# techshoww/RoMa

Measured on AMD Instinct MI355X. Metric: image-pairs/sec at 560->864, higher is better.
Workload: dtype fp16; 1 GPU; roma_outdoor 560->864 full coarse-to-fine symmetric match (BASELINE configs[1]; configs[2] = --pairs 8 --gpus 8); launch=eager launches, coarse_res=560, upsample_res=864, parallelism=single GPU

## Files before the change

include/roma_hip.h:

```cpp
#ifndef ROMA_HIP_H
#define ROMA_HIP_H

#include <stdint.h>

#ifdef __cplusplus
extern "C" {
#endif

#define ROMA_ABI_VERSION 5

enum { ROMA_F32 = 0, ROMA_F16 = 1, ROMA_BF16 = 2 };
enum { ROMA_NCHW = 0, ROMA_NHWC = 1 };
enum { ROMA_LC_AUTO = 0, ROMA_LC_TILE8X4 = 1, ROMA_LC_TILE8X8 = 2, ROMA_LC_ROWS8 = 3 };
enum { ROMA_E_ARG = -1, ROMA_E_DTYPE = -2, ROMA_E_SHAPE = -3, ROMA_E_ALIGN = -4, ROMA_E_UNSUPPORTED = -5 };

int roma_abi_version(void);
const char* roma_last_error(void);

int roma_local_corr(const void* f0, const void* f1, const float* flow, void* out,
                    int B, int C, int H, int W, int r, int dtype,
                    int layout, int f0_pitch, int f1_pitch, int out_layout, int out_pitch, int f1_batch_shift, int variant,
                    void* stream);

int roma_warp_bilinear(const void* src, const float* flow, void* dst,
                       int B, int C, int Hs, int Ws, int H, int W, int dtype,
                       int layout, int src_pitch, int dst_layout, int dst_pitch, int src_batch_shift, void* stream);

int roma_disp_emb(const float* flow, const float* weight, const float* bias, void* dst,
                  int B, int E, int H, int W, float gain, int dtype, int dst_layout, int dst_pitch, void* stream);

int roma_interp_bilinear(const float* x, float* y, int N, int Hi, int Wi, int Ho, int Wo, void* stream);

int roma_interp_bilinear_pair(const float* x0, float* y0, int N0, const float* x1, float* y1, int N1, int Hi, int Wi, int Ho, int Wo,
                              void* stream);

int roma_refiner_assemble(const void* src, const float* flow, const float* weight, const float* bias, void* buf, int B, int C, int E,
                          int D, int pitch, int Hs, int Ws, int H, int W, int src_pitch, int src_batch_shift, float gain, int dtype,
                          void* stream);

int roma_flow_update(float* flow, float* cert, const float* cert_in, const float* delta,
                     int B, int H, int W, float sx, float sy, void* stream);

int roma_cls_to_flow_refine(const void* logits, float* flow_out, float* cert_out,
                            int B, int C, int HW, long stride_b, long stride_c, long stride_p,
                            int dtype, void* stream);

int roma_cos_kernel(const void* x, const void* y, float* K, int B, int N, int M, int D, int dtype, int x_pitch, int y_pitch,
                    int y_batch_shift, float T, float eps, float diag_add, void* stream);

int roma_chol_diag_block(float* A, int lda, long strideA, float* W, int ldw, long strideW, int nb, int B, int* info,
                         int info_base, void* stream);

int roma_chol_step(float* A, int lda, long strideA, int n, int ncols, int j, int nb, const float* W, int ldw, long strideW, float* R,
                   int ldr, long strideR, float* Wn, int ldwn, long strideWn, int* info, int info_base, int B, void* stream);

int roma_chol_subst_step(int dir, const float* W, int ldw, long strideW, const float* R, long strideRb, long strideRs, int ldr, float* T,
                         long strideTb, long strideTs, int ldt, int t_in_panel, float* X, int ldx, long strideX, int n, int m, int nb,
                         int s, int B, void* stream);

int roma_attention_fwd(const void* q, const void* k, const void* v, void* o, int B, int H, int Nq, int Nk, int head_dim, long q_sb,
                       long q_sn, long q_sh, long k_sb, long k_sn, long k_sh, long v_sb, long v_sn, long v_sh, long o_sb, long o_sn,
                       long o_sh, float scale, int dtype, void* stream);

int roma_match_finalize(const float* flow, const float* cert, const float* cert16, float* warp, float* certainty,
                        int P, int H, int W, int H16, int W16, int symmetric, void* stream);

int roma_kde_density(const float* x, float* density, int N, int down, float std, int half_mode, void* stream);

int roma_race_keys(const float* p, const long* counter, float* keys, long N, float thresh, unsigned seed, unsigned stage,
                   void* stream);

int roma_nn_argmin(const float* q, const float* r, int* idx, int NQ, int NR, void* stream);

int roma_resample_u8(const void* in, void* out, int H, int W, int C, int out_size, int axis, const int* bounds,
                     const int* coef, int ksize, void* stream);
int roma_normalize_u8(const void* in, float* out, int H, int W, const float* mean3, const float* std3, void* stream);

int roma_bias_relu_nchw(void* x, const void* bias, int B, int C, int HW, int dtype, void* stream);

int roma_bias_relu_pool2_nchw(void* x, const void* bias, void* pooled, int B, int C, int H, int W, int dtype, void* stream);

int roma_bias_relu_nhwc(void* x, const void* bias, long npix, int C, int dtype, void* stream);
int roma_bias_relu_pool2_nhwc(void* x, const void* bias, void* pooled, int B, int C, int H, int W, int dtype, void* stream);

int roma_dwconv5x5_bn_relu(const void* x, const float* w, const float* scale, const float* shift, void* y,
                           int B, int C, int H, int W, int dtype, int x_pitch, int y_pitch, void* stream);

int roma_refiner_block(const void* x, const void* w25, const float* scale, const float* shift, const void* wt,
                       const float* bias, void* y, int B, int C, int H, int W, int kpad, int dtype, int x_pitch, int y_pitch,
                       void* stream);

int roma_refiner_wide_pack(const void* wt, void* wp, int D);
int roma_refiner_wide_taps(const void* w25, void* w25p, int D);
int roma_refiner_block_wide(const void* x, const void* w25p, const float* scale, const float* shift, const void* wp,
                            const float* bias, void* y, int B, int H, int W, int D, int x_pitch, int y_pitch, int dtype,
                            void* stream);

int roma_pointwise_mfma(const void* x, const void* wt, const float* bias, void* y, long M, int C, int kpad, int dtype,
                        int x_pitch, int y_pitch, void* stream);

int roma_refiner_head(const void* x, const float* wo, const float* bo, float* flow, const float* cert_in, float* cert_out,
// ... 76 lines not shown
```

roma_amd/_lib.py:

```python
from __future__ import annotations

import ctypes
import os
from ctypes import c_char_p, c_float, c_int, c_long, c_void_p

_HERE = os.path.dirname(os.path.abspath(__file__))
LIB_PATH = os.path.join(_HERE, "csrc", "libroma_hip.so")

ROMA_F32, ROMA_F16, ROMA_BF16 = 0, 1, 2
ROMA_NCHW, ROMA_NHWC = 0, 1
LC_VARIANTS = {"auto": 0, "tile8x4": 1, "tile8x8": 2, "rows8": 3}
ABI_VERSION = 5
SCORE_MSAC, SCORE_MAGSAC = 0, 1
ROMA_E_ARG, ROMA_E_DTYPE, ROMA_E_SHAPE, ROMA_E_ALIGN, ROMA_E_UNSUPPORTED = -1, -2, -3, -4, -5

SIGNATURES = {
    "roma_abi_version": [],
    "roma_last_error": [],
    "roma_local_corr": [c_void_p, c_void_p, c_void_p, c_void_p, c_int, c_int, c_int, c_int, c_int, c_int,
                        c_int, c_int, c_int, c_int, c_int, c_int, c_int, c_void_p],
    "roma_warp_bilinear": [c_void_p, c_void_p, c_void_p, c_int, c_int, c_int, c_int, c_int, c_int, c_int,
                           c_int, c_int, c_int, c_int, c_int, c_void_p],
    "roma_disp_emb": [c_void_p, c_void_p, c_void_p, c_void_p, c_int, c_int, c_int, c_int, c_float, c_int, c_int, c_int, c_void_p],
    "roma_interp_bilinear": [c_void_p, c_void_p, c_int, c_int, c_int, c_int, c_int, c_void_p],
    "roma_interp_bilinear_pair": [c_void_p, c_void_p, c_int, c_void_p, c_void_p, c_int, c_int, c_int, c_int, c_int, c_void_p],
    "roma_refiner_assemble": [c_void_p, c_void_p, c_void_p, c_void_p, c_void_p, c_int, c_int, c_int, c_int, c_int, c_int, c_int, c_int,
                              c_int, c_int, c_int, c_float, c_int, c_void_p],
    "roma_project_skinny": [c_void_p, c_void_p, c_void_p, c_void_p, c_long, c_int, c_int, c_int, c_int, c_int, c_void_p],
    "roma_flow_update": [c_void_p, c_void_p, c_void_p, c_void_p, c_int, c_int, c_int, c_float, c_float, c_void_p],
    "roma_cls_to_flow_refine": [c_void_p, c_void_p, c_void_p, c_int, c_int, c_int, c_long, c_long, c_long, c_int, c_void_p],
    "roma_cos_kernel": [c_void_p, c_void_p, c_void_p, c_int, c_int, c_int, c_int, c_int, c_int, c_int, c_int, c_float, c_float,
                        c_float, c_void_p],
    "roma_add_layernorm": [c_void_p, c_int, c_long, c_void_p, c_int, c_long, c_void_p, c_void_p, c_void_p, c_void_p, c_int, c_long,
                           c_long, c_int, c_float, c_void_p],
    "roma_attention_fwd": [c_void_p, c_void_p, c_void_p, c_void_p, c_int, c_int, c_int, c_int, c_int] + [c_long] * 12 + [c_float, c_int, c_void_p],
    "roma_chol_diag_block": [c_void_p, c_int, c_long, c_void_p, c_int, c_long, c_int, c_int, c_void_p, c_int, c_void_p],
    "roma_chol_step": [c_void_p, c_int, c_long, c_int, c_int, c_int, c_int, c_void_p, c_int, c_long, c_void_p, c_int, c_long,
                       c_void_p, c_int, c_long, c_void_p, c_int, c_int, c_void_p],
    "roma_chol_subst_step": [c_int, c_void_p, c_int, c_long, c_void_p, c_long, c_long, c_int, c_void_p, c_long, c_long, c_int, c_int,
                             c_void_p, c_int, c_long, c_int, c_int, c_int, c_int, c_int, c_void_p],
    "roma_match_finalize": [c_void_p, c_void_p, c_void_p, c_void_p, c_void_p, c_int, c_int, c_int, c_int, c_int, c_int, c_void_p],
    "roma_kde_density": [c_void_p, c_void_p, c_int, c_int, c_float, c_int, c_void_p],
    "roma_nn_argmin": [c_void_p, c_void_p, c_void_p, c_int, c_int, c_void_p],
    "roma_race_keys": [c_void_p, c_void_p, c_void_p, c_long, c_float, ctypes.c_uint, ctypes.c_uint, c_void_p],
    "roma_dwconv5x5_bn_relu": [c_void_p, c_void_p, c_void_p, c_void_p, c_void_p, c_int, c_int, c_int, c_int, c_int, c_int, c_int, c_void_p],
    "roma_resample_u8": [c_void_p, c_void_p, c_int, c_int, c_int, c_int, c_int, c_void_p, c_void_p, c_int, c_void_p],
    "roma_normalize_u8": [c_void_p, c_void_p, c_int, c_int, c_void_p, c_void_p, c_void_p],
    "roma_bias_relu_nchw": [c_void_p, c_void_p, c_int, c_int, c_int, c_int, c_void_p],
    "roma_bias_relu_pool2_nchw": [c_void_p, c_void_p, c_void_p, c_int, c_int, c_int, c_int, c_int, c_void_p],
    "roma_bias_relu_nhwc": [c_void_p, c_void_p, c_long, c_int, c_int, c_void_p],
    "roma_bias_relu_pool2_nhwc": [c_void_p, c_void_p, c_void_p, c_int, c_int, c_int, c_int, c_int, c_void_p],
    "roma_pointwise_mfma": [c_void_p, c_void_p, c_void_p, c_void_p, c_long, c_int, c_int, c_int, c_int, c_int, c_void_p],
    "roma_refiner_block": [c_void_p, c_void_p, c_void_p, c_void_p, c_void_p, c_void_p, c_void_p, c_int, c_int, c_int, c_int, c_int, c_int,
                           c_int, c_int, c_void_p],
    "roma_refiner_wide_pack": [c_void_p, c_void_p, c_int],
    "roma_refiner_wide_taps": [c_void_p, c_void_p, c_int],
    "roma_jpeg_info": [c_void_p, c_long, c_void_p],
    "roma_jpeg_entropy_decode": [c_void_p, c_long, c_void_p, c_void_p],
    "roma_jpeg_reconstruct": [c_void_p, c_void_p, c_void_p, c_void_p, c_void_p, c_void_p],
    "roma_refiner_block_wide": [c_void_p, c_void_p, c_void_p, c_void_p, c_void_p, c_void_p, c_void_p, c_int, c_int, c_int, c_int, c_int, c_int,
                                c_int, c_void_p],
    "roma_refiner_head": [c_void_p, c_void_p, c_void_p, c_void_p, c_void_p, c_void_p, c_void_p, c_int, c_int, c_int, c_int, c_int, c_int,
                          c_float, c_float, c_void_p],
    "roma_pointwise_small": [c_void_p, c_void_p, c_void_p, c_void_p, c_long, c_int, c_int, c_int, c_int, c_void_p],
    "roma_tiny_corr_posembed": [c_void_p, c_void_p, c_void_p, c_int, c_int, c_int, c_int, c_int, c_int, c_int, c_void_p],
    "roma_ransac_workspace": [c_int, c_int, c_int, c_int, c_void_p],
    "roma_ransac_hypotheses": [c_int, c_void_p, c_void_p, c_int, c_int, c_int, c_float, ctypes.c_uint, c_int, c_void_p, c_long, c_void_p],
    "roma_ransac_select": [c_int, c_void_p, c_void_p, c_int, c_int, c_int, c_float, c_int, c_void_p, c_long, c_void_p, c_void_p,
                           c_void_p],
    "roma_ransac_hypotheses_ex": [c_int, c_void_p, c_void_p, c_int, c_int, c_int, c_float, c_int, ctypes.c_uint, c_int, c_void_p, c_long,
                                  c_void_p],
    "roma_ransac_select_ex": [c_int, c_void_p, c_void_p, c_int, c_int, c_int, c_float, c_int, c_int, c_void_p, c_long, c_void_p, c_void_p,
                              c_void_p],
    "roma_magsac_table": [c_void_p, c_void_p],
    "roma_essential_workspace": [c_int, c_int, c_int, c_void_p],
    "roma_essential_hypotheses": [c_void_p, c_void_p, c_void_p, c_void_p, c_int, c_int, c_int, c_float, ctypes.c_uint, c_int, c_void_p,
                                  c_long, c_void_p],
    "roma_essential_select": [c_void_p, c_void_p, c_void_p, c_void_p, c_int, c_int, c_int, c_float, c_int, c_void_p, c_long, c_void_p,
                              c_void_p, c_void_p],
    "roma_essential_hypotheses_ex": [c_void_p, c_void_p, c_void_p, c_void_p, c_int, c_int, c_int, c_float, c_int, ctypes.c_uint, c_int,
                                     c_void_p, c_long, c_void_p],
    "roma_essential_select_ex": [c_void_p, c_void_p, c_void_p, c_void_p, c_int, c_int, c_int, c_float, c_int, c_int, c_void_p, c_long,
                                 c_void_p, c_void_p, c_void_p],
    "roma_recover_pose": [c_void_p, c_void_p, c_void_p, c_void_p, c_void_p, c_void_p, c_int, c_int, c_void_p, c_void_p, c_void_p,
                          c_void_p, c_void_p],
# ... 48 lines not shown
```

roma_amd/csrc/cos_kernel.hip:

```cpp
#include "common.h"

namespace roma {
namespace {

typedef float f32x16 __attribute__((ext_vector_type(16)));
constexpr int BT = 64, KT = 16, LD = KT + 1;

template <typename T> __device__ __forceinline__ float4_t ld4(const T* p) {
  if constexpr (sizeof(T) == 4) {
    return *reinterpret_cast<const float4_t*>(p);
  } else {
    typedef T v4 __attribute__((ext_vector_type(4)));
    const v4 h = *reinterpret_cast<const v4*>(p);
    return float4_t{(float)h[0], (float)h[1], (float)h[2], (float)h[3]};
  }
}

template <typename T>
__global__ __launch_bounds__(256) void cos_kernel_mfma(const T* __restrict__ x, const T* __restrict__ y, float* __restrict__ K,
                                                       int N, int M, int D, int x_pitch, int y_pitch, int y_shift, float invT,
                                                       float eps, float diag_add) {
  __shared__ float sA[BT * LD], sB[BT * LD];
  __shared__ double sN[2 * BT];
  const int tid = threadIdx.x, lane = tid & 63, wave = tid >> 6;
  const int wr = wave >> 1, wc = wave & 1;
  const int b = blockIdx.z, n0 = blockIdx.y * BT, m0 = blockIdx.x * BT;
  const T* xb = x + (size_t)b * N * x_pitch;
  const T* yb = y + (size_t)((b + y_shift) % (int)gridDim.z) * M * y_pitch;
  f32x16 acc;
  double accd[16];
#pragma unroll
  for (int i = 0; i < 16; ++i) { acc[i] = 0.f; accd[i] = 0.0; }
  double nrm = 0.0;
  const int lr = tid >> 2, lc = (tid & 3) * 4;
  for (int k0 = 0; k0 < D; k0 += KT) {
    float4_t va{0, 0, 0, 0}, vb{0, 0, 0, 0};
    if (n0 + lr < N) va = ld4<T>(xb + (size_t)(n0 + lr) * x_pitch + k0 + lc);
    if (m0 + lr < M) vb = ld4<T>(yb + (size_t)(m0 + lr) * y_pitch + k0 + lc);
    __syncthreads();
#pragma unroll
    for (int i = 0; i < 4; ++i) {
      sA[lr * LD + lc + i] = va[i];
      sB[lr * LD + lc + i] = vb[i];
    }
    __syncthreads();
    if (tid < 2 * BT) {
      const float* r = (tid < BT ? sA : sB) + (tid & (BT - 1)) * LD;
#pragma unroll
      for (int i = 0; i < KT; ++i) nrm = __builtin_fma((double)r[i], (double)r[i], nrm);
    }
    const float* pa = sA + (wr * 32 + (lane & 31)) * LD + (lane >> 5);
    const float* pb = sB + (wc * 32 + (lane & 31)) * LD + (lane >> 5);
#pragma unroll
    for (int kk = 0; kk < KT; kk += 2) acc = __builtin_amdgcn_mfma_f32_32x32x2f32(pa[kk], pb[kk], acc, 0, 0, 0);
    if (((k0 / KT) & 3) == 3 || k0 + KT >= D) {
#pragma unroll
      for (int i = 0; i < 16; ++i) { accd[i] += (double)acc[i]; acc[i] = 0.f; }
    }
  }
  if (tid < 2 * BT) sN[tid] = sqrt(nrm);
  __syncthreads();
  const int col = lane & 31;
  const int m = m0 + wc * 32 + col;
  const double ny = sN[BT + wc * 32 + col];
#pragma unroll
  for (int r = 0; r < 16; ++r) {
    const int row = (r & 3) + 8 * (r >> 2) + 4 * (lane >> 5);
    const int n = n0 + wr * 32 + row;
    if (n < N && m < M) {
      const double c = accd[r] / (sN[wr * 32 + row] * ny + (double)eps);
      float v = (float)exp((c - 1.0) * (double)invT);
      if (n == m) v += diag_add;
      K[((size_t)b * N + n) * M + m] = v;
    }
  }
}

}
}

using namespace roma;

extern "C" int roma_cos_kernel(const void* x, const void* y, float* K, int B, int N, int M, int D, int dtype, int x_pitch,
                               int y_pitch, int y_batch_shift, float T, float eps, float diag_add, void* stream) {
  ROMA_REQUIRE(x && y && K, ROMA_E_ARG, "roma_cos_kernel: null pointer");
  ROMA_REQUIRE(B > 0 && N > 0 && M > 0 && D > 0, ROMA_E_SHAPE, "roma_cos_kernel: bad shape");
  ROMA_REQUIRE(D % KT == 0, ROMA_E_SHAPE, "roma_cos_kernel: D=%d must be a multiple of %d", D, KT);
  ROMA_REQUIRE(x_pitch >= D && y_pitch >= D, ROMA_E_SHAPE, "roma_cos_kernel: row pitch smaller than D");
  ROMA_REQUIRE(dtype >= ROMA_F32 && dtype <= ROMA_BF16, ROMA_E_DTYPE, "roma_cos_kernel: unknown dtype %d", dtype);
  const int e16 = dtype == ROMA_F32 ? 4 : 8;
  ROMA_REQUIRE(aligned16(x) && aligned16(y) && x_pitch % e16 == 0 && y_pitch % e16 == 0, ROMA_E_ALIGN,
               "roma_cos_kernel: x and y must be 16-byte aligned with row pitches that keep every row 16-byte aligned");
  ROMA_REQUIRE(y_batch_shift >= 0 && y_batch_shift < B, ROMA_E_ARG, "roma_cos_kernel: y_batch_shift %d outside [0, B)", y_batch_shift);
  ROMA_REQUIRE(T > 0.f, ROMA_E_ARG, "roma_cos_kernel: temperature must be positive");
  dim3 grid((M + BT - 1) / BT, (N + BT - 1) / BT, B);
  hipStream_t s = static_cast<hipStream_t>(stream);
#define ROMA_COS(TT)                                                                                                         \
  hipLaunchKernelGGL((cos_kernel_mfma<TT>), grid, dim3(256), 0, s, (const TT*)x, (const TT*)y, K, N, M, D, x_pitch, y_pitch, \
                     y_batch_shift, 1.f / T, eps, diag_add)
  if (dtype == ROMA_F32) ROMA_COS(float); else if (dtype == ROMA_F16) ROMA_COS(half_t); else ROMA_COS(bf16_t);
#undef ROMA_COS
  ROMA_CHECK_LAUNCH();
}
```

roma_amd/matcher.py:

```python
from __future__ import annotations

import math
import os
from collections import namedtuple
from typing import Dict, Optional
from warnings import warn

import numpy as np
import torch
import torch.nn as nn
import torch.nn.functional as F

from . import ops
from .transformer import Block, TransformerDecoder

IMAGENET_MEAN = (0.485, 0.456, 0.406)
IMAGENET_STD = (0.229, 0.224, 0.225)


def pixel_grid(b, h, w, device):
    ys = torch.linspace(-1 + 1 / h, 1 - 1 / h, h, device=device)
    xs = torch.linspace(-1 + 1 / w, 1 - 1 / w, w, device=device)
    return torch.stack((xs[None, :].expand(h, w), ys[:, None].expand(h, w)), dim=0)[None].expand(b, 2, h, w).contiguous()

# ... 160 lines not shown
                cur = cur.view(B, h, w, Dp)
        return cur, P

    @torch.no_grad()
    def forward(self, x, y, flow, scale_factor=1, logits=None, dtype=None):
        flow = flow.float().contiguous()
        cur, P = self._body(x, y, flow, scale_factor, dtype or self.amp_dtype)
        B, h, w, Dp = cur.shape
        out = torch.addmm(P.bo, cur.reshape(B * h * w, Dp).float(), P.wo)
        out = out.view(B, h, w, self.out_dim).permute(0, 3, 1, 2).contiguous()
        return out[:, :-1], out[:, -1:]

    @torch.no_grad()
    def forward_update(self, x, y, flow, certainty, scale_factor, sx, sy, dtype=None, buf=None, batch_shift=0):
        cur, P = self._body(x, y, flow, scale_factor, dtype or self.amp_dtype, buf=buf, batch_shift=batch_shift)
        return ops.refiner_head(cur, P.wo, P.bo, flow, certainty, sx, sy)


class CosKernel(nn.Module):
    def __init__(self, T=0.2, learn_temperature=False):
        super().__init__()
        self.T = T

    def __call__(self, x, y, eps=1e-6):
        return ops.cos_kernel(x, y, T=self.T, eps=eps)


class GP(nn.Module):

    def __init__(self, gp_dim=512, T=0.2, sigma_noise=0.1, kernel=None, **_):
        super().__init__()
        self.K = CosKernel(T=T)
        self.sigma_noise = sigma_noise
        self.pos_conv = nn.Conv2d(2, gp_dim, 1, 1)
        self.dim = gp_dim
        self._basis = {}

    def basis(self, b, h, w, device):
        key = (h, w, device, _params_version(self.pos_conv))
        f = self._basis.get(key)
        if f is None:
            g = pixel_grid(1, h, w, device)
            f = torch.cos(8 * math.pi * F.conv2d(g, self.pos_conv.weight.float(), self.pos_conv.bias.float()))
            f = f.flatten(2).transpose(1, 2).contiguous()
            self._basis = {key: f}
        return f.expand(b, -1, -1)

    @torch.no_grad()
    def forward(self, x, y, **kwargs):
        b, c, h1, w1 = x.shape
        _, _, h2, w2 = y.shape
        xs = x.float().flatten(2).transpose(1, 2).contiguous()
        ys = y.float().flatten(2).transpose(1, 2).contiguous()
        K_yy = ops.cos_kernel(ys, ys, T=self.K.T, diag_add=self.sigma_noise)
        K_xy = ops.cos_kernel(xs, ys, T=self.K.T)
        mu = self.posterior_product(K_xy, ops.spd_solve(K_yy, self.basis(1, h2, w2, x.device)))
        return mu.transpose(1, 2).reshape(b, self.dim, h1, w1)

    def posterior_rows(self, xs, ys, h2, w2, fp64=False, batch_shift=0, out=None, check="now"):
        B, n = xs.shape[0], xs.shape[1]
        s = batch_shift % B
        basis = self.basis(1, h2, w2, xs.device)
        if fp64:
            a = xs.double()
            c = (a.roll(-s, 0) if s else a) if ys is None else ys.double()

            def cosk(u, v):
                g = torch.einsum("bnd,bmd->bnm", u, v) / (u.norm(dim=-1)[..., None] * v.norm(dim=-1)[:, None] + 1e-6)
                return ((g - 1.0) / self.K.T).exp()

            Kyy = cosk(c, c) + self.sigma_noise * torch.eye(c.shape[1], device=c.device, dtype=torch.float64)
            Z = torch.cholesky_solve(basis.double().expand(B, -1, -1), torch.linalg.cholesky(Kyy))
            mu = (cosk(a, c) @ Z).float()
            if out is not None:
                out.copy_(mu)
                return out
            return mu
        if ys is None:
            K_self = ops.cos_kernel(xs, xs, T=self.K.T, diag_add=self.sigma_noise)
            K_xy = ops.cos_kernel(xs, xs, T=self.K.T, batch_shift=s)
            Z = ops.spd_solve(K_self, basis, check=check)
            if s:
                assert 2 * s == B, "only the half swap of forward_symmetric"
                Z = torch.cat((Z[s:], Z[:s]), dim=0)
        else:
            K_yy = ops.cos_kernel(ys, ys, T=self.K.T, diag_add=self.sigma_noise)
            K_xy = ops.cos_kernel(xs, ys, T=self.K.T)
            Z = ops.spd_solve(K_yy, basis, check=check)
        return self.posterior_product(K_xy, Z, out)

    @staticmethod
    def posterior_product(K_xy, Z, out=None):
        mu = torch.bmm(K_xy.double(), Z.double())
        if out is None:
            return mu.float()
        out.copy_(mu)
        return out


class Decoder(nn.Module):
    def __init__(self, embedding_decoder, gps, proj, conv_refiner, detach=True, scales=("16", "8", "4", "2", "1"),
                 amp_dtype=torch.float16, **_):
        super().__init__()
        self.embedding_decoder, self.gps, self.proj, self.conv_refiner = embedding_decoder, gps, proj, conv_refiner
        self.scales = list(scales)
        self.refine_init = 4
        self.amp_dtype = amp_dtype
        self.gp_precision = "fp32"
        self.record = None
        self.flow_override = None
        self._proj = None

    def _embedding_decoder_for(self, dtype):
        if dtype == torch.float32:
            return self.embedding_decoder
        key = (dtype, _params_version(self.embedding_decoder))
        hit = self.__dict__.get("_embed_cast")
        if hit is None or hit[0] != key:
            import copy
            with torch.inference_mode(False), torch.no_grad():
                cp = copy.deepcopy(self.embedding_decoder).eval()
                for m in cp.modules():
                    if isinstance(m, nn.Linear):
                        m.to(dtype)
                hit = (key, cp)
            self.__dict__["_embed_cast"] = hit
        return hit[1]

    def get_placeholder_flow(self, b, h, w, device):
        return pixel_grid(b, h, w, device)

    def folded_proj(self, dtype):
        key = (dtype, _params_version(self.proj))
        if self._proj is not None and self._proj[0] == key:
            return self._proj[1]
        out = {}
        for s, seq in self.proj.items():
            conv, bn = seq[0], seq[1]
            g = bn.weight.float() / torch.sqrt(bn.running_var.float() + bn.eps)
            wt = (conv.weight.float().reshape(conv.out_channels, -1) * g[:, None]).t().contiguous().to(dtype)
            b = ((conv.bias.float() - bn.running_mean.float()) * g + bn.bias.float()).to(dtype)
            out[s] = (wt, b)
# ... 370 lines not shown
```

roma_amd/ops.py:

```python
from __future__ import annotations

import math
from typing import Optional

import torch

from . import _lib
from ._lib import ROMA_BF16, ROMA_F16, ROMA_F32, ROMA_NCHW, ROMA_NHWC, check

_DT = {torch.float32: ROMA_F32, torch.float16: ROMA_F16, torch.bfloat16: ROMA_BF16}


class KernelTimer:

    def __init__(self):
        self.enabled = False
        self.bracket_overhead_s = 0.0
        self.records = []

    def start(self):
        self.records.clear()
        torch.cuda.synchronize()
        pairs = []
        for _ in range(32):
            s, e = torch.cuda.Event(enable_timing=True), torch.cuda.Event(enable_timing=True)
            s.record()
            e.record()
            pairs.append((s, e))
        torch.cuda.synchronize()
        gaps = sorted(s.elapsed_time(e) * 1e-3 for s, e in pairs)
        self.bracket_overhead_s = gaps[len(gaps) // 2]
        self.enabled = True

    def stop(self):
        self.enabled = False

    def wrap(self, name, nbytes, tag, launch):
        if not self.enabled or torch.cuda.is_current_stream_capturing():
            return launch()
        s, e = torch.cuda.Event(enable_timing=True), torch.cuda.Event(enable_timing=True)
        s.record()
        out = launch()
        e.record()
        self.records.append((name, nbytes, s, e, tag))
        return out

    def summary(self):
        out = {}
        for name, nbytes, s, e, tag in self.records:
            d = out.setdefault(name, {"launches": 0, "bytes": 0, "seconds": 0.0, "by_tag": {}})
            t = max(s.elapsed_time(e) * 1e-3 - self.bracket_overhead_s, 1e-7)
            d["launches"] += 1
            d["bytes"] += nbytes
            d["seconds"] += t
            bt = d["by_tag"].setdefault(tag, [0, 0, 0.0])
            bt[0] += 1
            bt[1] += nbytes
            bt[2] += t
        return out


TIMER = KernelTimer()


def _need_gpu(*ts):
    dev = None
    for t in ts:
        if t is None:
            continue
        if not t.is_cuda:
            raise RuntimeError("roma_amd kernels run on an MI355X (ROCm device tensors) only; got a "
                               f"{t.device} tensor and there is no CPU fallback")
        if dev is None:
            dev = t.device
        elif t.device != dev:
            raise RuntimeError(f"roma_amd kernel arguments live on different devices ({dev} and {t.device})")
    if dev is not None and dev.index != torch.cuda.current_device():
        raise RuntimeError(f"roma_amd kernel arguments live on {dev} but the current device is cuda:{torch.cuda.current_device()}; "
                           "wrap the call in `with torch.cuda.device(t.device):`")


def _stream():
    return torch.cuda.current_stream().cuda_stream


def _dt(t):
    try:
        return _DT[t.dtype]
    except KeyError:
        raise ValueError(f"unsupported dtype {t.dtype}") from None


def _p(t):
    return None if t is None else t.data_ptr()


def feat_layout(t: torch.Tensor):
    B, C, H, W = t.shape
    sb, sc, sh, sw = t.stride()
    if sc == 1 and sh == W * sw and sb == H * W * sw and sw >= C:
        return ROMA_NHWC, sw, t
    if t.is_contiguous():
        return ROMA_NCHW, C, t
    t = t.contiguous()
    return ROMA_NCHW, C, t


def nhwc_empty(B, C, H, W, dtype, device, pitch=None):
    pitch = pitch or C
    buf = torch.empty((B, H, W, pitch), dtype=dtype, device=device)
    return buf[..., :C].permute(0, 3, 1, 2)


def local_correlation(feature0, feature1, local_radius, padding_mode="zeros", flow=None, sample_mode="bilinear", out=None,
                      batch_shift=0, variant="auto"):
# ... 113 lines not shown
    check(_lib.load().roma_flow_update(_p(flow), _p(cert), _p(cert_in), _p(delta), B, H, W, float(sx), float(sy), _stream()),
          "roma_flow_update")
    return flow, cert


def cls_to_flow_refine(cls):
    _need_gpu(cls)
    B, C, H, W = cls.shape
    sb, sc, sh, sw = cls.stride()
    if sh != W * sw:
        cls = cls.contiguous()
        sb, sc, sh, sw = cls.stride()
    flow = torch.empty((B, 2, H, W), dtype=torch.float32, device=cls.device)
    check(_lib.load().roma_cls_to_flow_refine(_p(cls), _p(flow), None, B, C, H * W, sb, sc, sw, _dt(cls), _stream()),
          "roma_cls_to_flow_refine")
    return flow.permute(0, 2, 3, 1)


def cls_rows_to_flow(rows, B, H, W):
    _need_gpu(rows)
    assert rows.dim() == 3 and rows.shape[0] == B and rows.shape[1] == H * W and rows.stride(2) == 1
    C = rows.shape[2] - 1
    flow = torch.empty((B, 2, H, W), dtype=torch.float32, device=rows.device)
    cert = torch.empty((B, 1, H, W), dtype=torch.float32, device=rows.device)
    check(_lib.load().roma_cls_to_flow_refine(_p(rows), _p(flow), _p(cert), B, C, H * W, rows.stride(0), 1, rows.stride(1),
                                              _dt(rows), _stream()), "roma_cls_to_flow_refine")
    return flow, cert


def _rows(t):
    B, N, D = t.shape
    es = t.element_size()
    if t.stride(2) == 1 and t.stride(0) == N * t.stride(1) and t.stride(1) >= D and (t.stride(1) * es) % 16 == 0 \
            and t.data_ptr() % 16 == 0 and t.dtype in _DT:
        return t, t.stride(1)
    t = (t if t.dtype in _DT else t.float()).contiguous()
    return t, D


def cos_kernel(x, y, T=0.2, eps=1e-6, diag_add=0.0, batch_shift=0):
    _need_gpu(x, y)
    if x.dtype != y.dtype:
        x, y = x.float(), y.float()
    x, xp = _rows(x)
    y, yp = _rows(y)
    B, N, D = x.shape
    M = y.shape[1]
    K = torch.empty((B, N, M), dtype=torch.float32, device=x.device)
    check(_lib.load().roma_cos_kernel(_p(x), _p(y), _p(K), B, N, M, D, _dt(x), xp, yp, int(batch_shift) % B, float(T), float(eps),
                                      float(diag_add), _stream()), "roma_cos_kernel")
    return K


class _PendingSpdCheck:

    def __init__(self, info):
        self.host = torch.empty(info.shape, dtype=info.dtype, pin_memory=True)
        self.host.copy_(info, non_blocking=True)
        self.event = torch.cuda.Event()
        self.event.record()

    def result(self):
        self.event.synchronize()
        return self.host.tolist()


_PENDING = []


def _raise_if_not_spd(bad):
    if any(bad):
        b = next(i for i, v in enumerate(bad) if v)
        raise _lib.RomaHipError(f"spd_solve: matrix {b} of the batch is not positive definite (block step {(bad[b] - 1) // 64}, pivot "
                                f"{(bad[b] - 1) % 64} is <= 0 or NaN) — non-finite or degenerate features?  The reference's "
                                f"torch.linalg.inv raises here too (matcher.py:261).")


_DEFER_DEPTH = [0]


def deferring():
    return _DEFER_DEPTH[0] > 0


class deferred_spd_checks:

    def __enter__(self):
        _DEFER_DEPTH[0] += 1
        return self

    def __exit__(self, et, ev, tb):
        _DEFER_DEPTH[0] -= 1
        if _DEFER_DEPTH[0] > 0:
            return False
        todo, _PENDING[:] = list(_PENDING), []
        if et is None and not torch.cuda.is_current_stream_capturing():
            for chk in todo:
                _raise_if_not_spd(chk.result())
        return False


def raise_pending():
    if torch.cuda.is_current_stream_capturing():
        return
    todo, _PENDING[:] = list(_PENDING), []
    for chk in todo:
        _raise_if_not_spd(chk.result())


def spd_solve(K, F, check="now", refine=0):
    _need_gpu(K, F)
    assert K.dtype == torch.float32 and F.dtype == torch.float32
    tun = torch.cuda.tunable.is_enabled()
    if tun:
        torch.cuda.tunable.enable(False)
    try:
        X, info = _spd_solve(K, F, refine)
    finally:
        if tun:
            torch.cuda.tunable.enable(True)
    if check == "now":
        _raise_if_not_spd(info.tolist())
    elif check == "defer":
        _PENDING.append(_PendingSpdCheck(info))
    return X


def _spd_solve(K, F, refine=0):
    nb = 64
    B, n, _ = K.shape
    m = F.shape[2]
    lib = _lib.load()
    A = torch.cat((K, F.expand(B, -1, -1)), dim=2)
    steps = [(j, min(j + nb, n)) for j in range(0, n, nb)]
    W = torch.empty((B, len(steps), nb, nb), dtype=torch.float32, device=K.device)
    info = torch.zeros((B,), dtype=torch.int32, device=K.device)
    Rall = torch.empty((B, len(steps), nb, n + m), dtype=torch.float32, device=K.device)
    check(lib.roma_chol_diag_block(A.data_ptr(), A.stride(1), A.stride(0), W.data_ptr(), nb, W.stride(0), steps[0][1], B,
                                   info.data_ptr(), 0, _stream()), "roma_chol_diag_block")
    for s, (j, e) in enumerate(steps):
        last = s + 1 == len(steps)
        check(lib.roma_chol_step(A.data_ptr(), A.stride(1), A.stride(0), n, n + m, j, e - j, W[:, s].data_ptr(), nb, W.stride(0),
                                 Rall[:, s].data_ptr(), n + m, Rall.stride(0), None if last else W[:, s + 1].data_ptr(), nb, W.stride(0),
                                 info.data_ptr(), nb * (s + 1), B, _stream()), "roma_chol_step")
    X = torch.empty((B, n, m), dtype=torch.float32, device=K.device)
    S = len(steps)

    def subst(direction, T, sTb, sTs, ldt, in_panel, out):
        for s in (range(S - 1, -1, -1) if direction < 0 else range(S)):
            check(lib.roma_chol_subst_step(direction, W[:, s].data_ptr(), nb, W.stride(0), Rall.data_ptr(), Rall.stride(0), Rall.stride(1),
                                           n + m, T.data_ptr(), sTb, sTs, ldt, in_panel, out.data_ptr(), m, out.stride(0), n, m, nb, s, B,
                                           _stream()), "roma_chol_subst_step")

    subst(-1, Rall, Rall.stride(0), Rall.stride(1), n + m, 1, X)
    for _ in range(int(refine)):
        g = (F.double() - torch.bmm(K.double(), X.double())).float().contiguous()
        y = torch.empty_like(g)
        subst(+1, g, g.stride(0), nb * m, m, 0, y)
        d = torch.empty_like(g)
        subst(-1, y, y.stride(0), nb * m, m, 0, d)
        X = X + d
    return X, info


def match_finalize(flow, certainty, cert16, symmetric=True):
    _need_gpu(flow, certainty, cert16)
    B, _, H, W = flow.shape
    P = B // 2 if symmetric else B
    flow = flow.float().contiguous()
    certainty = certainty.float().contiguous()
    H16 = W16 = 0
    if cert16 is not None:
        cert16 = cert16.float().contiguous()
        H16, W16 = cert16.shape[-2:]
    WW = 2 * W if symmetric else W
    warp = torch.empty((P, H, WW, 4), dtype=torch.float32, device=flow.device)
    cert = torch.empty((P, H, WW), dtype=torch.float32, device=flow.device)
    check(_lib.load().roma_match_finalize(_p(flow), _p(certainty), _p(cert16), _p(warp), _p(cert), P, H, W, H16, W16,
                                          1 if symmetric else 0, _stream()), "roma_match_finalize")
    return warp, cert


def kde(x, std=0.1, half=True, down=None):
    _need_gpu(x)
    if x.dim() != 2 or x.shape[1] != 4:
        raise ValueError("kde expects (N,4) matches")
    xs = (x.half() if half else x).float().contiguous()
    N = xs.shape[0]
    dens = torch.empty((N,), dtype=torch.float32, device=x.device)
    check(_lib.load().roma_kde_density(_p(xs), _p(dens), N, int(down or 1), float(std), 1 if half else 0, _stream()), "roma_kde_density")
    return dens.half() if half else dens


def race_keys(p, thresh=-1.0, seed=0, counter=None, stage=0):
    _need_gpu(p, counter)
    p = p.reshape(-1).float().contiguous()
    if counter is not None:
        counter = counter.reshape(-1).long().contiguous()
        assert counter.numel() == p.numel()
    keys = torch.empty_like(p)
    check(_lib.load().roma_race_keys(_p(p), _p(counter), _p(keys), p.numel(), float(thresh), int(seed) & 0xFFFFFFFF,
                                     int(stage) & 0xFFFFFFFF, _stream()), "roma_race_keys")
    return keys


def nn_argmin(q, r):
    _need_gpu(q, r)
    if q.dim() != 2 or q.shape[1] != 2 or r.dim() != 2 or r.shape[1] != 2:
        raise ValueError("nn_argmin expects (N,2) point sets")
    q, r = q.float().contiguous(), r.float().contiguous()
    idx = torch.empty((q.shape[0],), dtype=torch.int32, device=q.device)
    check(_lib.load().roma_nn_argmin(_p(q), _p(r), _p(idx), q.shape[0], r.shape[0], _stream()), "roma_nn_argmin")
    return idx.long()


# ... 221 lines not shown
```

Baseline: 59.10 image-pairs/s.

## Fuse GP kernel matrices into one launch writing directly into Cholesky buffer

```diff
diff --git a/include/roma_hip.h b/include/roma_hip.h
--- a/include/roma_hip.h
+++ b/include/roma_hip.h
@@ -47,6 +47,10 @@
 
 int roma_cos_kernel(const void* x, const void* y, float* K, int B, int N, int M, int D, int dtype, int x_pitch, int y_pitch,
                     int y_batch_shift, float T, float eps, float diag_add, void* stream);
+
+int roma_gp_kernel_matrices(const void* x, const void* y, float* Kyy, long kyy_pitch, long kyy_bstride, void* Kxy, int kxy_f64,
+                            double* norms, int B, int N, int M, int D, int dtype, int x_pitch, int y_pitch, int y_batch_shift,
+                            int mirror, float T, float eps, float diag_add, void* stream);
 
 int roma_chol_diag_block(float* A, int lda, long strideA, float* W, int ldw, long strideW, int nb, int B, int* info,
                          int info_base, void* stream);
diff --git a/roma_amd/_lib.py b/roma_amd/_lib.py
--- a/roma_amd/_lib.py
+++ b/roma_amd/_lib.py
@@ -31,6 +31,8 @@
     "roma_cls_to_flow_refine": [c_void_p, c_void_p, c_void_p, c_int, c_int, c_int, c_long, c_long, c_long, c_int, c_void_p],
     "roma_cos_kernel": [c_void_p, c_void_p, c_void_p, c_int, c_int, c_int, c_int, c_int, c_int, c_int, c_int, c_float, c_float,
                         c_float, c_void_p],
+    "roma_gp_kernel_matrices": [c_void_p, c_void_p, c_void_p, c_long, c_long, c_void_p, c_int, c_void_p, c_int, c_int, c_int, c_int,
+                                c_int, c_int, c_int, c_int, c_int, c_float, c_float, c_float, c_void_p],
     "roma_add_layernorm": [c_void_p, c_int, c_long, c_void_p, c_int, c_long, c_void_p, c_void_p, c_void_p, c_void_p, c_int, c_long,
                            c_long, c_int, c_float, c_void_p],
     "roma_attention_fwd": [c_void_p, c_void_p, c_void_p, c_void_p, c_int, c_int, c_int, c_int, c_int] + [c_long] * 12 + [c_float, c_int, c_void_p],
diff --git a/roma_amd/csrc/cos_kernel.hip b/roma_amd/csrc/cos_kernel.hip
--- a/roma_amd/csrc/cos_kernel.hip
+++ b/roma_amd/csrc/cos_kernel.hip
@@ -74,6 +74,189 @@
       K[((size_t)b * N + n) * M + m] = v;
     }
   }
+}
+
+struct GPParams {
+  const void* x; const void* y;
+  float* Kyy; long kyy_pitch, kyy_bstride;
+  void* Kxy;
+  const double* nx; const double* ny;
+  int B, N, M, D, x_pitch, y_pitch, shift, mirror, kxy_f64;
+  int Tn, Tm, self_jobs, kyy_vec, kxy_vec;
+  float invT, eps, diag_add;
+};
+
+typedef double double2_t __attribute__((ext_vector_type(2)));
+
+__device__ __forceinline__ void st4(float* p, const float* v) { *reinterpret_cast<float4_t*>(p) = float4_t{v[0], v[1], v[2], v[3]}; }
+__device__ __forceinline__ void st4(double* p, const float* v) {
+  *reinterpret_cast<double2_t*>(p) = double2_t{(double)v[0], (double)v[1]};
+  *reinterpret_cast<double2_t*>(p + 2) = double2_t{(double)v[2], (double)v[3]};
+}
+
+template <typename O>
+__device__ __forceinline__ void store_direct(O* out, long pitch, const float* v, int r0, int c, int half, int R, int C) {
+  if (c >= C) return;
+#pragma unroll
+  for (int r = 0; r < 16; ++r) {
+    const int row = r0 + (r & 3) + 8 * (r >> 2) + 4 * half;
+    if (row < R) out[(size_t)row * pitch + c] = (O)v[r];
+  }
+}
+template <typename O>
+__device__ __forceinline__ void store_transposed(O* out, long pitch, const float* v, int r0, int c, int half, int R, int C, bool vec) {
+  if (c >= C) return;
+#pragma unroll
+  for (int g = 0; g < 4; ++g) {
+    const int row = r0 + 8 * g + 4 * half;
+    O* p = out + (size_t)c * pitch + row;
+    if (vec && row + 3 < R) {
+      st4(p, v + 4 * g);
+    } else {
+#pragma unroll
+      for (int i = 0; i < 4; ++i)
+        if (row + i < R) p[i] = (O)v[4 * g + i];
+    }
+  }
+}
+
+template <typename T, bool PRE>
+__global__ __launch_bounds__(256) void gp_kernel_matrices_kernel(const GPParams p) {
+  __shared__ float sA[BT * LD], sB[BT * LD];
+  __shared__ double sN[2 * BT];
+  const int tid = threadIdx.x, lane = tid & 63, wave = tid >> 6;
+  const int wr = wave >> 1, wc = wave & 1;
+  int job = blockIdx.x, b, n0, m0;
+  const bool self = job < p.self_jobs;
+  if (self) {
+    const int tri = p.Tm * (p.Tm + 1) / 2;
+    b = job / tri;
+    int t = job - b * tri, i = 0;
+    while (t >= p.Tm - i) { t -= p.Tm - i; ++i; }
+    n0 = i * BT;
+    m0 = (i + t) * BT;
+  } else {
+    job -= p.self_jobs;
+    const int per = p.Tn * p.Tm;
+    b = job / per;
+    const int t = job - b * per;
+    n0 = (t / p.Tm) * BT;
+    m0 = (t % p.Tm) * BT;
+  }
+  const int by = (b + p.shift) % p.B;
+  const int N = self ? p.M : p.N, M = p.M, D = p.D;
+  const int x_pitch = self ? p.y_pitch : p.x_pitch, y_pitch = p.y_pitch;
+  const T* yb = (const T*)p.y + (size_t)by * M * y_pitch;
+  const T* xb = self ? yb : (const T*)p.x + (size_t)b * N * x_pitch;
+  if constexpr (PRE) {
+    if (tid < 2 * BT) {
+      const int i = tid & (BT - 1);
+      double v = 0.0;
+      if (tid < BT) { if (n0 + i < N) v = self ? p.ny[(size_t)by * M + n0 + i] : p.nx[(size_t)b * N + n0 + i]; }
+      else if (m0 + i < M) v = p.ny[(size_t)by * M + m0 + i];
+      sN[tid] = v;
+    }
+  }
+  f32x16 acc;
+  double accd[16];
+#pragma unroll
+  for (int i = 0; i < 16; ++i) { acc[i] = 0.f; accd[i] = 0.0; }
+  double nrm = 0.0;
+  const int lr = tid >> 2, lc = (tid & 3) * 4;
+  const bool in_a = n0 + lr < N, in_b = m0 + lr < M;
+  const T* ga = xb + (size_t)(n0 + lr) * x_pitch + lc;
+  const T* gb = yb + (size_t)(m0 + lr) * y_pitch + lc;
+  float4_t va{0, 0, 0, 0}, vb{0, 0, 0, 0};
+  if (in_a) va = ld4<T>(ga);
+  if (in_b) vb = ld4<T>(gb);
+  for (int k0 = 0; k0 < D; k0 += KT) {
+    __syncthreads();
+#pragma unroll
+    for (int i = 0; i < 4; ++i) {
+      sA[lr * LD + lc + i] = va[i];
+      sB[lr * LD + lc + i] = vb[i];
+    }
+    __syncthreads();
+    if (k0 + KT < D) {
+      if (in_a) va = ld4<T>(ga + k0 + KT);
+      if (in_b) vb = ld4<T>(gb + k0 + KT);
+    }
+    if constexpr (!PRE) {
+      if (tid < 2 * BT) {
+        const float* r = (tid < BT ? sA : sB) + (tid & (BT - 1)) * LD;
+#pragma unroll
+        for (int i = 0; i < KT; ++i) nrm = __builtin_fma((double)r[i], (double)r[i], nrm);
+      }
+    }
+    const float* pa = sA + (wr * 32 + (lane & 31)) * LD + (lane >> 5);
+    const float* pb = sB + (wc * 32 + (lane & 31)) * LD + (lane >> 5);
+#pragma unroll
+    for (int kk = 0; kk < KT; kk += 2) acc = __builtin_amdgcn_mfma_f32_32x32x2f32(pa[kk], pb[kk], acc, 0, 0, 0);
+    if (((k0 / KT) & 3) == 3 || k0 + KT >= D) {
+#pragma unroll
+      for (int i = 0; i < 16; ++i) { accd[i] += (double)acc[i]; acc[i] = 0.f; }
+    }
+  }
+  if constexpr (!PRE) {
+    if (tid < 2 * BT) sN[tid] = sqrt(nrm);
+  }
+  __syncthreads();
+  const int col = lane & 31, half = lane >> 5;
+  const int m = m0 + wc * 32 + col;
+  const double ny = sN[BT + wc * 32 + col];
+  float v[16];
+#pragma unroll
+  for (int r = 0; r < 16; ++r) {
+    const int row = (r & 3) + 8 * (r >> 2) + 4 * half;
+    const double c = accd[r] / (sN[wr * 32 + row] * ny + (double)p.eps);
+    v[r] = (float)exp((c - 1.0) * (double)p.invT);
+    if (self && n0 + wr * 32 + row == m) v[r] += p.diag_add;
+  }
+  const int r0 = n0 + wr * 32;
+  if (self) {
+    float* out = p.Kyy + (size_t)b * p.kyy_bstride;
+    store_direct(out, p.kyy_pitch, v, r0, m, half, N, M);
+    if (n0 != m0) store_transposed(out, p.kyy_pitch, v, r0, m, half, N, M, p.kyy_vec != 0);
+  } else if (p.kxy_f64) {
+    double* out = (double*)p.Kxy + (size_t)b * N * M;
+    store_direct(out, (long)M, v, r0, m, half, N, M);
+    if (p.mirror) store_transposed(out + (size_t)p.shift * N * M, (long)N, v, r0, m, half, N, M, p.kxy_vec != 0);
+  } else {
+    float* out = (float*)p.Kxy + (size_t)b * N * M;
+    store_direct(out, (long)M, v, r0, m, half, N, M);
+    if (p.mirror) store_transposed(out + (size_t)p.shift * N * M, (long)N, v, r0, m, half, N, M, p.kxy_vec != 0);
+  }
+}
+
+constexpr int NC = 64, NLD = NC + 1;
+template <typename T>
+__global__ __launch_bounds__(256) void row_norm_kernel(const T* __restrict__ x, double* __restrict__ out, long rows, int D, int pitch) {
+  __shared__ float s[BT * NLD];
+  const int tid = threadIdx.x, lr = tid >> 2, lc = (tid & 3) * 4;
+  const long row0 = (long)blockIdx.x * BT;
+  const bool in = row0 + lr < rows;
+  const T* g = x + (size_t)(row0 + lr) * pitch + lc;
+  float4_t v[4];
+#pragma unroll
+  for (int j = 0; j < 4; ++j) v[j] = (in && lc + 16 * j < D) ? ld4<T>(g + 16 * j) : float4_t{0, 0, 0, 0};
+  double nrm = 0.0;
+  for (int k0 = 0; k0 < D; k0 += NC) {
+    __syncthreads();
+#pragma unroll
+    for (int j = 0; j < 4; ++j)
+#pragma unroll
+      for (int i = 0; i < 4; ++i) s[lr * NLD + lc + 16 * j + i] = v[j][i];
+    __syncthreads();
+#pragma unroll
+    for (int j = 0; j < 4; ++j)
+      if (in && k0 + NC + lc + 16 * j < D) v[j] = ld4<T>(g + k0 + NC + 16 * j);
+    if (tid < BT) {
+      const float* r = s + tid * NLD;
+      const int kn = D - k0 < NC ? D - k0 : NC;
+      for (int i = 0; i < kn; ++i) nrm = __builtin_fma((double)r[i], (double)r[i], nrm);
+    }
+  }
+  if (tid < BT && row0 + tid < rows) out[row0 + tid] = sqrt(nrm);
 }
 
 }
@@ -102,3 +285,58 @@
 #undef ROMA_COS
   ROMA_CHECK_LAUNCH();
 }
+
+extern "C" int roma_gp_kernel_matrices(const void* x, const void* y, float* Kyy, long kyy_pitch, long kyy_bstride, void* Kxy,
+                                       int kxy_f64, double* norms, int B, int N, int M, int D, int dtype, int x_pitch, int y_pitch,
+                                       int y_batch_shift, int mirror, float T, float eps, float diag_add, void* stream) {
+  ROMA_REQUIRE(y && (Kyy || Kxy) && (x || !Kxy), ROMA_E_ARG, "roma_gp_kernel_matrices: null pointer");
+  ROMA_REQUIRE(B > 0 && N > 0 && M > 0 && D > 0, ROMA_E_SHAPE, "roma_gp_kernel_matrices: bad shape");
+  ROMA_REQUIRE(D % KT == 0, ROMA_E_SHAPE, "roma_gp_kernel_matrices: D=%d must be a multiple of %d", D, KT);
+  ROMA_REQUIRE(x_pitch >= D && y_pitch >= D, ROMA_E_SHAPE, "roma_gp_kernel_matrices: row pitch smaller than D");
+  ROMA_REQUIRE(dtype >= ROMA_F32 && dtype <= ROMA_BF16, ROMA_E_DTYPE, "roma_gp_kernel_matrices: unknown dtype %d", dtype);
+  const int e16 = dtype == ROMA_F32 ? 4 : 8;
+  ROMA_REQUIRE((!Kxy || aligned16(x)) && aligned16(y) && x_pitch % e16 == 0 && y_pitch % e16 == 0, ROMA_E_ALIGN,
+               "roma_gp_kernel_matrices: x and y must be 16-byte aligned with row pitches that keep every row 16-byte aligned");
+  ROMA_REQUIRE(y_batch_shift >= 0 && y_batch_shift < B, ROMA_E_ARG, "roma_gp_kernel_matrices: y_batch_shift %d outside [0, B)",
+               y_batch_shift);
+  ROMA_REQUIRE(T > 0.f, ROMA_E_ARG, "roma_gp_kernel_matrices: temperature must be positive");
+  ROMA_REQUIRE(!Kyy || (kyy_pitch >= M && kyy_bstride >= (long)(M - 1) * kyy_pitch + M), ROMA_E_SHAPE,
+               "roma_gp_kernel_matrices: K_yy pitch %ld / batch stride %ld too small for %d x %d", kyy_pitch, kyy_bstride, M, M);
+  ROMA_REQUIRE(!mirror || (Kxy && x == y && N == M && x_pitch == y_pitch && 2 * y_batch_shift == B), ROMA_E_ARG,
+               "roma_gp_kernel_matrices: mirrored cross tiles need y = x and 2 * y_batch_shift = B");
+  ROMA_REQUIRE(!norms || (reinterpret_cast<uintptr_t>(norms) & 7) == 0, ROMA_E_ALIGN, "roma_gp_kernel_matrices: norms misaligned");
+  GPParams p;
+  p.x = x; p.y = y; p.Kyy = Kyy; p.kyy_pitch = kyy_pitch; p.kyy_bstride = kyy_bstride; p.Kxy = Kxy;
+  p.B = B; p.N = N; p.M = M; p.D = D; p.x_pitch = x_pitch; p.y_pitch = y_pitch; p.shift = y_batch_shift; p.mirror = mirror ? 1 : 0;
+  p.kxy_f64 = kxy_f64 ? 1 : 0;
+  p.Tn = (N + BT - 1) / BT; p.Tm = (M + BT - 1) / BT;
+  p.self_jobs = Kyy ? B * (p.Tm * (p.Tm + 1) / 2) : 0;
+  p.kyy_vec = Kyy && aligned16(Kyy) && kyy_pitch % 4 == 0 && kyy_bstride % 4 == 0;
+  p.kxy_vec = Kxy && aligned16(Kxy) && N % 4 == 0;
+  p.invT = 1.f / T; p.eps = eps; p.diag_add = diag_add;
+  const long cross_jobs = Kxy ? (long)(mirror ? B / 2 : B) * p.Tn * p.Tm : 0;
+  ROMA_REQUIRE(p.self_jobs + cross_jobs < (1l << 31), ROMA_E_SHAPE, "roma_gp_kernel_matrices: too many tiles");
+  hipStream_t s = static_cast<hipStream_t>(stream);
+  const bool x_is_y = x == y && N == M && x_pitch == y_pitch;
+  p.ny = norms;
+  p.nx = !norms ? nullptr : (x_is_y ? norms : norms + (size_t)B * M);
+  const bool need_nx = norms && Kxy && !x_is_y;
+  dim3 grid((unsigned)(p.self_jobs + cross_jobs));
+#define ROMA_GP(TT)                                                                                                              \
+  do {                                                                                                                           \
+    if (norms) {                                                                                                                 \
+      const long ry = (long)B * M, rx = (long)B * N;                                                                             \
+      hipLaunchKernelGGL((row_norm_kernel<TT>), dim3((unsigned)((ry + BT - 1) / BT)), dim3(256), 0, s, (const TT*)y, norms, ry,  \
+                         D, y_pitch);                                                                                            \
+      if (need_nx)                                                                                                               \
+        hipLaunchKernelGGL((row_norm_kernel<TT>), dim3((unsigned)((rx + BT - 1) / BT)), dim3(256), 0, s, (const TT*)x,           \
+                           norms + ry, rx, D, x_pitch);                                                                          \
+      hipLaunchKernelGGL((gp_kernel_matrices_kernel<TT, true>), grid, dim3(256), 0, s, p);                                       \
+    } else {                                                                                                                     \
+      hipLaunchKernelGGL((gp_kernel_matrices_kernel<TT, false>), grid, dim3(256), 0, s, p);                                      \
+    }                                                                                                                            \
+  } while (0)
+  if (dtype == ROMA_F32) ROMA_GP(float); else if (dtype == ROMA_F16) ROMA_GP(half_t); else ROMA_GP(bf16_t);
+#undef ROMA_GP
+  ROMA_CHECK_LAUNCH();
+}
diff --git a/roma_amd/matcher.py b/roma_amd/matcher.py
--- a/roma_amd/matcher.py
+++ b/roma_amd/matcher.py
@@ -236,10 +236,18 @@
         _, _, h2, w2 = y.shape
         xs = x.float().flatten(2).transpose(1, 2).contiguous()
         ys = y.float().flatten(2).transpose(1, 2).contiguous()
-        K_yy = ops.cos_kernel(ys, ys, T=self.K.T, diag_add=self.sigma_noise)
-        K_xy = ops.cos_kernel(xs, ys, T=self.K.T)
-        mu = self.posterior_product(K_xy, ops.spd_solve(K_yy, self.basis(1, h2, w2, x.device)))
+        mu = self._posterior(xs, ys, 0, self.basis(1, h2, w2, x.device), "now", None)
         return mu.transpose(1, 2).reshape(b, self.dim, h1, w1)
+
+    def _posterior(self, xs, ys, s, basis, check, out):
+        B = xs.shape[0]
+        n, m = basis.shape[1], basis.shape[2]
+        A = torch.empty((B, n, n + m), dtype=torch.float32, device=xs.device)
+        A[:, :, n:].copy_(basis)
+        _, K_xy = ops.gp_kernel_matrices(xs, ys, T=self.K.T, diag_add=self.sigma_noise, batch_shift=s, kyy_out=A[:, :, :n],
+                                         kxy_dtype=torch.float64)
+        Z = ops.spd_solve_augmented(A, n, check=check, batch_shift=s)
+        return self.posterior_product(K_xy, Z, out)
 
     def posterior_rows(self, xs, ys, h2, w2, fp64=False, batch_shift=0, out=None, check="now"):
         B, n = xs.shape[0], xs.shape[1]
@@ -260,18 +268,7 @@
                 out.copy_(mu)
                 return out
             return mu
-        if ys is None:
-            K_self = ops.cos_kernel(xs, xs, T=self.K.T, diag_add=self.sigma_noise)
-            K_xy = ops.cos_kernel(xs, xs, T=self.K.T, batch_shift=s)
-            Z = ops.spd_solve(K_self, basis, check=check)
-            if s:
-                assert 2 * s == B, "only the half swap of forward_symmetric"
-                Z = torch.cat((Z[s:], Z[:s]), dim=0)
-        else:
-            K_yy = ops.cos_kernel(ys, ys, T=self.K.T, diag_add=self.sigma_noise)
-            K_xy = ops.cos_kernel(xs, ys, T=self.K.T)
-            Z = ops.spd_solve(K_yy, basis, check=check)
-        return self.posterior_product(K_xy, Z, out)
+        return self._posterior(xs, ys, s if ys is None else 0, basis, check, out)
 
     @staticmethod
     def posterior_product(K_xy, Z, out=None):
diff --git a/roma_amd/ops.py b/roma_amd/ops.py
--- a/roma_amd/ops.py
+++ b/roma_amd/ops.py
@@ -61,6 +61,8 @@
 
 
 TIMER = KernelTimer()
+
+GP_ROW_NORM_PREPASS = False
 
 
 def _need_gpu(*ts):
@@ -280,9 +282,51 @@
     return K
 
 
+def gp_kernel_matrices(x, y=None, T=0.2, eps=1e-6, diag_add=0.0, batch_shift=0, kyy_out=None, kxy_dtype=torch.float32,
+                       kxy_out=None, want_kyy=True, want_kxy=True, row_norms=None):
+    _need_gpu(x, y, kyy_out, kxy_out)
+    if kxy_out is not None:
+        kxy_dtype = kxy_out.dtype
+    if y is not None and x.dtype != y.dtype:
+        x, y = x.float(), y.float()
+    x, xp = _rows(x)
+    if y is None:
+        y, yp = x, xp
+    else:
+        y, yp = _rows(y)
+    B, N, D = x.shape
+    M = y.shape[1]
+    if y.shape[0] != B or y.shape[2] != D:
+        raise ValueError(f"gp_kernel_matrices: x {tuple(x.shape)} and y {tuple(y.shape)} do not match")
+    if kxy_dtype not in (torch.float32, torch.float64):
+        raise ValueError(f"gp_kernel_matrices: kxy_dtype {kxy_dtype} is neither fp32 nor fp64")
+    s = int(batch_shift) % B
+    K_yy = K_xy = None
+    pitch = bstride = 0
+    if want_kyy:
+        K_yy = torch.empty((B, M, M), dtype=torch.float32, device=x.device) if kyy_out is None else kyy_out
+        if K_yy.dtype != torch.float32 or tuple(K_yy.shape) != (B, M, M) or K_yy.stride(2) != 1:
+            raise ValueError("gp_kernel_matrices: kyy_out must be a (B,M,M) fp32 view with unit column stride")
+        pitch, bstride = K_yy.stride(1), K_yy.stride(0)
+    if want_kxy:
+        K_xy = torch.empty((B, N, M), dtype=kxy_dtype, device=x.device) if kxy_out is None else kxy_out
+        if tuple(K_xy.shape) != (B, N, M) or not K_xy.is_contiguous():
+            raise ValueError("gp_kernel_matrices: kxy_out must be a contiguous (B,N,M) tensor")
+    same = y.data_ptr() == x.data_ptr() and N == M and xp == yp
+    mirror = bool(want_kxy and same and s > 0 and 2 * s == B)
+    norms = None
+    if GP_ROW_NORM_PREPASS if row_norms is None else row_norms:
+        norms = torch.empty((B * (N + M),), dtype=torch.float64, device=x.device)
+    check(_lib.load().roma_gp_kernel_matrices(_p(x), _p(y), _p(K_yy), pitch, bstride, _p(K_xy), int(kxy_dtype == torch.float64),
+                                              _p(norms), B, N, M, D, _dt(x), xp, yp, s, int(mirror), float(T), float(eps),
+                                              float(diag_add), _stream()), "roma_gp_kernel_matrices")
+    return K_yy, K_xy
+
+
 class _PendingSpdCheck:
 
-    def __init__(self, info):
+    def __init__(self, info, batch_shift=0):
+        self.batch_shift = batch_shift
         self.host = torch.empty(info.shape, dtype=info.dtype, pin_memory=True)
         self.host.copy_(info, non_blocking=True)
         self.event = torch.cuda.Event()
@@ -296,11 +340,12 @@
 _PENDING = []
 
 
-def _raise_if_not_spd(bad):
+def _raise_if_not_spd(bad, batch_shift=0):
     if any(bad):
-        b = next(i for i, v in enumerate(bad) if v)
-        raise _lib.RomaHipError(f"spd_solve: matrix {b} of the batch is not positive definite (block step {(bad[b] - 1) // 64}, pivot "
-                                f"{(bad[b] - 1) % 64} is <= 0 or NaN) — non-finite or degenerate features?  The reference's "
+        i = next(i for i, v in enumerate(bad) if v)
+        b = (i + batch_shift) % len(bad)
+        raise _lib.RomaHipError(f"spd_solve: matrix {b} of the batch is not positive definite (block step {(bad[i] - 1) // 64}, pivot "
+                                f"{(bad[i] - 1) % 64} is <= 0 or NaN) — non-finite or degenerate features?  The reference's "
                                 f"torch.linalg.inv raises here too (matcher.py:261).")
 
 
@@ -324,7 +369,7 @@
         todo, _PENDING[:] = list(_PENDING), []
         if et is None and not torch.cuda.is_current_stream_capturing():
             for chk in todo:
-                _raise_if_not_spd(chk.result())
+                _raise_if_not_spd(chk.result(), chk.batch_shift)
         return False
 
 
@@ -333,7 +378,7 @@
         return
     todo, _PENDING[:] = list(_PENDING), []
     for chk in todo:
-        _raise_if_not_spd(chk.result())
+        _raise_if_not_spd(chk.result(), chk.batch_shift)
 
 
 def spd_solve(K, F, check="now", refine=0):
@@ -347,40 +392,31 @@
     finally:
         if tun:
             torch.cuda.tunable.enable(True)
+    _spd_check(info, check, 0)
+    return X
+
+
+def spd_solve_augmented(A, n, check="now", batch_shift=0):
+    _need_gpu(A)
+    if A.dtype != torch.float32 or A.dim() != 3 or not A.is_contiguous() or A.shape[1] != n or A.shape[2] <= n:
+        raise ValueError(f"spd_solve_augmented: A must be a contiguous (B, n, n+m) fp32 buffer with m > 0, got {tuple(A.shape)}")
+    X, info = _spd_solve_augmented(A, n)
+    _spd_check(info, check, int(batch_shift) % A.shape[0])
+    return X
+
+
+def _spd_check(info, check, batch_shift):
     if check == "now":
-        _raise_if_not_spd(info.tolist())
+        _raise_if_not_spd(info.tolist(), batch_shift)
     elif check == "defer":
-        _PENDING.append(_PendingSpdCheck(info))
-    return X
+        _PENDING.append(_PendingSpdCheck(info, batch_shift))
 
 
 def _spd_solve(K, F, refine=0):
-    nb = 64
     B, n, _ = K.shape
     m = F.shape[2]
-    lib = _lib.load()
-    A = torch.cat((K, F.expand(B, -1, -1)), dim=2)
-    steps = [(j, min(j + nb, n)) for j in range(0, n, nb)]
-    W = torch.empty((B, len(steps), nb, nb), dtype=torch.float32, device=K.device)
-    info = torch.zeros((B,), dtype=torch.int32, device=K.device)
-    Rall = torch.empty((B, len(steps), nb, n + m), dtype=torch.float32, device=K.device)
-    check(lib.roma_chol_diag_block(A.data_ptr(), A.stride(1), A.stride(0), W.data_ptr(), nb, W.stride(0), steps[0][1], B,
-                                   info.data_ptr(), 0, _stream()), "roma_chol_diag_block")
-    for s, (j, e) in enumerate(steps):
-        last = s + 1 == len(steps)
-        check(lib.roma_chol_step(A.data_ptr(), A.stride(1), A.stride(0), n, n + m, j, e - j, W[:, s].data_ptr(), nb, W.stride(0),
-                                 Rall[:, s].data_ptr(), n + m, Rall.stride(0), None if last else W[:, s + 1].data_ptr(), nb, W.stride(0),
-                                 info.data_ptr(), nb * (s + 1), B, _stream()), "roma_chol_step")
-    X = torch.empty((B, n, m), dtype=torch.float32, device=K.device)
-    S = len(steps)
-
-    def subst(direction, T, sTb, sTs, ldt, in_panel, out):
-        for s in (range(S - 1, -1, -1) if direction < 0 else range(S)):
-            check(lib.roma_chol_subst_step(direction, W[:, s].data_ptr(), nb, W.stride(0), Rall.data_ptr(), Rall.stride(0), Rall.stride(1),
-                                           n + m, T.data_ptr(), sTb, sTs, ldt, in_panel, out.data_ptr(), m, out.stride(0), n, m, nb, s, B,
-                                           _stream()), "roma_chol_subst_step")
-
-    subst(-1, Rall, Rall.stride(0), Rall.stride(1), n + m, 1, X)
+    nb = 64
+    X, info, subst = _spd_solve_augmented(torch.cat((K, F.expand(B, -1, -1)), dim=2), n, want_subst=True)
     for _ in range(int(refine)):
         g = (F.double() - torch.bmm(K.double(), X.double())).float().contiguous()
         y = torch.empty_like(g)
@@ -389,6 +425,35 @@
         subst(-1, y, y.stride(0), nb * m, m, 0, d)
         X = X + d
     return X, info
+
+
+def _spd_solve_augmented(A, n, want_subst=False):
+    nb = 64
+    B = A.shape[0]
+    m = A.shape[2] - n
+    lib = _lib.load()
+    steps = [(j, min(j + nb, n)) for j in range(0, n, nb)]
+    W = torch.empty((B, len(steps), nb, nb), dtype=torch.float32, device=A.device)
+    info = torch.zeros((B,), dtype=torch.int32, device=A.device)
+    Rall = torch.empty((B, len(steps), nb, n + m), dtype=torch.float32, device=A.device)
+    check(lib.roma_chol_diag_block(A.data_ptr(), A.stride(1), A.stride(0), W.data_ptr(), nb, W.stride(0), steps[0][1], B,
+                                   info.data_ptr(), 0, _stream()), "roma_chol_diag_block")
+    for s, (j, e) in enumerate(steps):
+        last = s + 1 == len(steps)
+        check(lib.roma_chol_step(A.data_ptr(), A.stride(1), A.stride(0), n, n + m, j, e - j, W[:, s].data_ptr(), nb, W.stride(0),
+                                 Rall[:, s].data_ptr(), n + m, Rall.stride(0), None if last else W[:, s + 1].data_ptr(), nb, W.stride(0),
+                                 info.data_ptr(), nb * (s + 1), B, _stream()), "roma_chol_step")
+    X = torch.empty((B, n, m), dtype=torch.float32, device=A.device)
+    S = len(steps)
+
+    def subst(direction, T, sTb, sTs, ldt, in_panel, out):
+        for s in (range(S - 1, -1, -1) if direction < 0 else range(S)):
+            check(lib.roma_chol_subst_step(direction, W[:, s].data_ptr(), nb, W.stride(0), Rall.data_ptr(), Rall.stride(0), Rall.stride(1),
+                                           n + m, T.data_ptr(), sTb, sTs, ldt, in_panel, out.data_ptr(), m, out.stride(0), n, m, nb, s, B,
+                                           _stream()), "roma_chol_subst_step")
+
+    subst(-1, Rall, Rall.stride(0), Rall.stride(1), n + m, 1, X)
+    return (X, info, subst) if want_subst else (X, info)
 
 
 def match_finalize(flow, certainty, cert16, symmetric=True):
```

Result: no change. 59.54 image-pairs/s, median of 6 (+0.7%).
